# dmMaze/comic-text-detector

Hardware: AMD Instinct MI355X
Metric: pages/sec at 1024x1024 bs=32 (end-to-end detector, device-resident pages) (higher is better)
Workload: dtype f16

## Files before the change

### comic-text-detector_amd/csrc/kernels.h

```cpp
#pragma once
#include <vector>

#include "ctd_common.h"
#include "tuning.h"

void launch_conv_direct(const ConvArgs& a, bool f16, hipStream_t st);
void launch_convt_direct(const ConvArgs& a, bool f16, hipStream_t st);
void launch_input_nchw(const float* in, void* dst, int pitch, int B, int H, int W, bool f16, hipStream_t st);
void launch_input_u8(const uint8_t* in, void* dst, int pitch, int B, int H, int W, bool f16, hipStream_t st);
void launch_maxpool(const void* src, int pitchS, void* dst, int pitchD, int C, int B, int H, int W, int k,
                    bool f16, hipStream_t st);
bool sppf_pool3_supported(int pitch, int slot, int C, int H, int W, int k, const void* cat, int esize = 2);
void launch_sppf_pool3(void* cat, int pitch, int slot, int C, int B, int H, int W, int k, hipStream_t st, int esize = 2);
void launch_avgpool2(const void* src, int pitchS, void* dst, int pitchD, int C, int B, int Ho, int Wo,
                     bool f16, hipStream_t st);
void launch_detect_decode(const void* raw, int pitch, bool raw_f16, float* blks, int rows_total, int row_off,
                          int B, int ny, int nx, int na, int no, float stride, const float* anchors_px,
                          hipStream_t st);
void launch_export_plane(const void* src, int pitch, bool f16, float* out, int nplanes, int plane, uint8_t* u8,
                         int u8_mode, float thresh, int B, int H, int W, hipStream_t st);

void launch_db_step(const float* lines, float k, float* out, uint8_t* bitmap, float thresh, int B, int H, int W,
                    hipStream_t st);

extern int g_igemm_force_bk;
int igemm_pick_bk(int c0, int c1, int K, int N, int log2_down);
void igemm_pack_weights(const float* logical, int nphase, int N, int K, int bn, int bk, bool tiled,
                        std::vector<half_t>& out);
bool igemm_supported(const ConvArgs& a);
int igemm_ntile(int N);
const char* launch_conv_igemm(const ConvArgs& a, bool dst_f32, hipStream_t st);

int f32_mfma_ntile(int N);
bool conv_f32_mfma_supported(const ConvArgs& a);
void launch_conv_f32_mfma(const ConvArgs& a, hipStream_t st);

bool conv_split_supported(const ConvArgs& a);
const char* launch_conv_split(const ConvArgs& a, hipStream_t st);
bool stem_split_supported(const ConvArgs& a);
void launch_stem_split(const ConvArgs& a, const void* input, int in_fmt, hipStream_t st);
bool conv_split_halo_supported(const ConvArgs& a);
void launch_conv_split_halo(const ConvArgs& a, hipStream_t st);
void split_pack_weights(const float* logical, int nphase, int N, int K, int npad, std::vector<half_t>& out,
                        std::vector<float>& oscale);

bool conv_halo_supported(const ConvArgs& a, bool dst_f32);
void launch_conv_halo(const ConvArgs& a, hipStream_t st);

bool conv_halo3_supported(const ConvArgs& a, bool dst_f32);
bool conv_halo3_post_supported(const ConvArgs& a);
bool conv_halo3_segp_supported(const ConvArgs& a);
void launch_conv_halo3(const ConvArgs& a, hipStream_t st);

struct C3Args {
  SrcView s0, s1;
  int B, H, W;
  const half_t *w12, *wm1, *wm2, *wc3;
  const float *b12, *bm1, *bm2, *bc3;
// ... 99 lines not shown
```

### comic-text-detector_amd/csrc/kernels_basic.hip

```cpp
#include "kernels.h"

namespace {

template <typename T>
__device__ __forceinline__ const T* src_pixel(const SrcView& s, int b, int iy, int ix) {
  int sy = s.up ? (iy >> 1) : iy;
  int sx = s.up ? (ix >> 1) : ix;
  return (const T*)s.ptr + ((size_t)((size_t)b * s.H + sy) * s.W + sx) * s.pitch;
}

template <typename T, bool PRECISE>
__global__ __launch_bounds__(256) void conv_direct_kernel(ConvArgs a) {
  const long long total = (long long)a.M * a.N;
  const int Ct = a.s0.c + a.s1.c;
  const float* __restrict__ w = (const float*)a.w;
  for (long long idx = (long long)blockIdx.x * blockDim.x + threadIdx.x; idx < total;
       idx += (long long)gridDim.x * blockDim.x) {
    const int n = (int)(idx % a.N);
    const int m = (int)(idx / a.N);
    const int ox = m % a.Mw;
    const int oy = (m / a.Mw) % a.Mh;
    const int b = m / (a.Mw * a.Mh);
    float acc = 0.f;
    for (int ty = 0; ty < a.KH; ++ty) {
// ... 108 lines not shown
    dst[pix * pitchD + c] = from_f<T>(m);
  }
}

__global__ void maxpool_h8_kernel(const half_t* __restrict__ src, int pitchS, half_t* __restrict__ dst, int pitchD,
                                  int C8, int B, int H, int W, int k) {
  const long long total = (long long)B * H * W * C8;
  const int r = k / 2;
  for (long long i = (long long)blockIdx.x * blockDim.x + threadIdx.x; i < total;
       i += (long long)gridDim.x * blockDim.x) {
    const int c = (int)(i % C8) * 8;
    const long long pix = i / C8;
    const int x = (int)(pix % W), y = (int)((pix / W) % H);
    const long long b = pix / ((long long)W * H);
    half8_t m;
#pragma unroll
    for (int e = 0; e < 8; ++e) m[e] = (half_t)-65504.f;
    for (int dy = -r; dy <= r; ++dy) {
      const int yy = y + dy;
      if (yy < 0 || yy >= H) continue;
      for (int dx = -r; dx <= r; ++dx) {
        const int xx = x + dx;
        if (xx < 0 || xx >= W) continue;
        const half8_t v = *(const half8_t*)(src + ((b * H + yy) * W + xx) * pitchS + c);
#pragma unroll
        for (int e = 0; e < 8; ++e) m[e] = v[e] > m[e] ? v[e] : m[e];
      }
    }
    *(half8_t*)(dst + pix * pitchD + c) = m;
  }
}

constexpr int SPPF_LDS_BYTES = 65536;
template <typename T, typename V, int NV>
__global__ __launch_bounds__(256) void sppf_pool3_kernel(T* __restrict__ cat, int pitch, int slot, int CG, int H, int W, int r) {
  __shared__ __attribute__((aligned(16))) unsigned char sm_raw[SPPF_LDS_BYTES];
  V* A = (V*)sm_raw;
  V* Bf = A + H * W;
  const int HW = H * W;
  const int b = blockIdx.x / CG, cg = blockIdx.x - b * CG;
  T* base = cat + (size_t)b * HW * pitch + cg * NV;
  for (int p = threadIdx.x; p < HW; p += 256) A[p] = *(const V*)(base + (size_t)p * pitch);
  __syncthreads();
  auto vmax = [](V a, V b2) {
    V o;
#pragma unroll
    for (int e = 0; e < NV; ++e) o[e] = b2[e] > a[e] ? b2[e] : a[e];
    return o;
  };
  for (int lvl = 1; lvl <= 3; ++lvl) {
    for (int p = threadIdx.x; p < HW; p += 256) {
      const int y = p / W, x = p - y * W;
      V m = A[p];
      for (int dx = -r; dx <= r; ++dx)
        if (dx && (unsigned)(x + dx) < (unsigned)W) m = vmax(m, A[p + dx]);
      Bf[p] = m;
    }
    __syncthreads();
    for (int p = threadIdx.x; p < HW; p += 256) {
      const int y = p / W;
      V m = Bf[p];
      for (int dy = -r; dy <= r; ++dy)
        if (dy && (unsigned)(y + dy) < (unsigned)H) m = vmax(m, Bf[p + dy * W]);
      A[p] = m;
      *(V*)(base + (size_t)lvl * slot + (size_t)p * pitch) = m;
    }
    __syncthreads();
  }
}

template <typename T>
__global__ void avgpool2_kernel(const T* __restrict__ src, int pitchS, T* __restrict__ dst, int pitchD, int C,
                                int B, int Ho, int Wo) {
  const long long total = (long long)B * Ho * Wo * C;
  const int Wi = Wo * 2, Hi = Ho * 2;
  for (long long i = (long long)blockIdx.x * blockDim.x + threadIdx.x; i < total;
       i += (long long)gridDim.x * blockDim.x) {
    const int c = (int)(i % C);
    const long long pix = i / C;
    const int x = (int)(pix % Wo), y = (int)((pix / Wo) % Ho);
    const long long b = pix / ((long long)Wo * Ho);
    const T* p = src + ((b * Hi + 2 * y) * Wi + 2 * x) * pitchS + c;
    const float s = (to_f(p[0]) + to_f(p[pitchS])) + (to_f(p[(size_t)Wi * pitchS]) + to_f(p[(size_t)(Wi + 1) * pitchS]));
    dst[pix * pitchD + c] = from_f<T>(s * 0.25f);
  }
}

template <typename T>
__global__ void detect_decode_kernel(const T* __restrict__ raw, int pitch, float* __restrict__ blks, int rows_total,
                                     int row_off, int B, int ny, int nx, int na, int no, float stride,
                                     const float* __restrict__ anchors) {
  const long long total = (long long)B * na * ny * nx;
  for (long long i = (long long)blockIdx.x * blockDim.x + threadIdx.x; i < total;
       i += (long long)gridDim.x * blockDim.x) {
    const int x = (int)(i % nx), y = (int)((i / nx) % ny);
    const int an = (int)((i / ((long long)nx * ny)) % na);
    const long long b = i / ((long long)nx * ny * na);
    const T* p = raw + ((b * ny + y) * nx + x) * pitch + an * no;
    float* o = blks + (b * rows_total + row_off + ((long long)an * ny + y) * nx + x) * no;
    for (int j = 0; j < no; ++j) {
      const float s = 1.0f / (1.0f + expf(-to_f(p[j])));
      float v = s;
      if (j == 0) v = (s * 2.f - 0.5f + (float)x) * stride;
      else if (j == 1) v = (s * 2.f - 0.5f + (float)y) * stride;
      else if (j == 2) { const float t = s * 2.f; v = t * t * anchors[an * 2 + 0]; }
      else if (j == 3) { const float t = s * 2.f; v = t * t * anchors[an * 2 + 1]; }
      o[j] = v;
    }
  }
}

template <typename T>
__global__ void export_plane_kernel(const T* __restrict__ src, int pitch, float* __restrict__ out, int nplanes,
                                    int plane, uint8_t* __restrict__ u8, int u8_mode, float thresh, int B, int H,
                                    int W) {
  const long long hw = (long long)H * W;
  const long long total = (long long)B * hw;
  for (long long i = (long long)blockIdx.x * blockDim.x + threadIdx.x; i < total;
       i += (long long)gridDim.x * blockDim.x) {
    const long long b = i / hw, p = i % hw;
    const float v = to_f(src[i * pitch]);
    if (out) out[(b * nplanes + plane) * hw + p] = v;
    if (u8_mode == 1) u8[i] = (uint8_t)(v * 255.0f);
    else if (u8_mode == 2) u8[i] = v > thresh ? 1 : 0;
  }
}

inline int grid_for(long long total, int block = 256) {
  long long g = (total + block - 1) / block;
  if (g > 256LL * 32) g = 256LL * 32;
  if (g < 1) g = 1;
  return (int)g;
}

}

void launch_conv_direct(const ConvArgs& a, bool f16, hipStream_t st) {
  const int g = grid_for((long long)a.M * a.N);
  if (f16) hipLaunchKernelGGL((conv_direct_kernel<half_t, false>), dim3(g), dim3(256), 0, st, a);
  else hipLaunchKernelGGL((conv_direct_kernel<float, true>), dim3(g), dim3(256), 0, st, a);
// ... 6 lines not shown
}

void launch_input_nchw(const float* in, void* dst, int pitch, int B, int H, int W, bool f16, hipStream_t st) {
  const int g = grid_for((long long)B * H * W);
  if (f16) hipLaunchKernelGGL((input_nchw_kernel<half_t>), dim3(g), dim3(256), 0, st, in, (half_t*)dst, pitch, B, H, W);
  else hipLaunchKernelGGL((input_nchw_kernel<float>), dim3(g), dim3(256), 0, st, in, (float*)dst, pitch, B, H, W);
}

void launch_input_u8(const uint8_t* in, void* dst, int pitch, int B, int H, int W, bool f16, hipStream_t st) {
  const long long t = (long long)B * H * W;
  const int g = grid_for(t);
  if (f16) hipLaunchKernelGGL((input_u8_kernel<half_t>), dim3(g), dim3(256), 0, st, in, (half_t*)dst, pitch, t);
  else hipLaunchKernelGGL((input_u8_kernel<float>), dim3(g), dim3(256), 0, st, in, (float*)dst, pitch, t);
}

void launch_maxpool(const void* src, int pitchS, void* dst, int pitchD, int C, int B, int H, int W, int k,
                    bool f16, hipStream_t st) {
  const int g = grid_for((long long)B * H * W * C);
  if (f16 && C % 8 == 0 && pitchS % 8 == 0 && pitchD % 8 == 0 && (((uintptr_t)src | (uintptr_t)dst) & 15) == 0)
    hipLaunchKernelGGL(maxpool_h8_kernel, dim3(grid_for((long long)B * H * W * (C / 8))), dim3(256), 0, st,
                       (const half_t*)src, pitchS, (half_t*)dst, pitchD, C / 8, B, H, W, k);
  else if (f16)
    hipLaunchKernelGGL((maxpool_kernel<half_t>), dim3(g), dim3(256), 0, st, (const half_t*)src, pitchS,
                       (half_t*)dst, pitchD, C, B, H, W, k);
  else
    hipLaunchKernelGGL((maxpool_kernel<float>), dim3(g), dim3(256), 0, st, (const float*)src, pitchS, (float*)dst,
                       pitchD, C, B, H, W, k);
}

bool sppf_pool3_supported(int pitch, int slot, int C, int H, int W, int k, const void* cat, int esize) {
  if (k != 5 && k != 3 && k != 7) return false;
  const int v = 16 / esize;
  if (C % v || pitch % v || slot % v || ((uintptr_t)cat & 15)) return false;
  return (long long)H * W * 2 * 8 <= SPPF_LDS_BYTES;
}
void launch_sppf_pool3(void* cat, int pitch, int slot, int C, int B, int H, int W, int k, hipStream_t st, int esize) {
  typedef float float2_t __attribute__((ext_vector_type(2)));
  const bool wide = (long long)H * W * 2 * 16 <= SPPF_LDS_BYTES;
  if (esize == 4) {
    if (wide)
      hipLaunchKernelGGL((sppf_pool3_kernel<float, float4_t, 4>), dim3(B * (C / 4)), dim3(256), 0, st, (float*)cat, pitch, slot, C / 4, H, W, k / 2);
    else
      hipLaunchKernelGGL((sppf_pool3_kernel<float, float2_t, 2>), dim3(B * (C / 2)), dim3(256), 0, st, (float*)cat, pitch, slot, C / 2, H, W, k / 2);
  } else if (wide) {
    hipLaunchKernelGGL((sppf_pool3_kernel<half_t, half8_t, 8>), dim3(B * (C / 8)), dim3(256), 0, st, (half_t*)cat, pitch, slot, C / 8, H, W, k / 2);
  } else {
    hipLaunchKernelGGL((sppf_pool3_kernel<half_t, half4_t, 4>), dim3(B * (C / 4)), dim3(256), 0, st, (half_t*)cat, pitch, slot, C / 4, H, W, k / 2);
  }
}

void launch_avgpool2(const void* src, int pitchS, void* dst, int pitchD, int C, int B, int Ho, int Wo, bool f16,
                     hipStream_t st) {
  const int g = grid_for((long long)B * Ho * Wo * C);
  if (f16)
    hipLaunchKernelGGL((avgpool2_kernel<half_t>), dim3(g), dim3(256), 0, st, (const half_t*)src, pitchS,
                       (half_t*)dst, pitchD, C, B, Ho, Wo);
  else
    hipLaunchKernelGGL((avgpool2_kernel<float>), dim3(g), dim3(256), 0, st, (const float*)src, pitchS, (float*)dst,
                       pitchD, C, B, Ho, Wo);
}

void launch_detect_decode(const void* raw, int pitch, bool raw_f16, float* blks, int rows_total, int row_off, int B,
                          int ny, int nx, int na, int no, float stride, const float* anchors_px, hipStream_t st) {
  const int g = grid_for((long long)B * na * ny * nx);
  if (raw_f16)
    hipLaunchKernelGGL((detect_decode_kernel<half_t>), dim3(g), dim3(256), 0, st, (const half_t*)raw, pitch, blks,
                       rows_total, row_off, B, ny, nx, na, no, stride, anchors_px);
  else
    hipLaunchKernelGGL((detect_decode_kernel<float>), dim3(g), dim3(256), 0, st, (const float*)raw, pitch, blks,
                       rows_total, row_off, B, ny, nx, na, no, stride, anchors_px);
}

__global__ void db_step_kernel(const float* __restrict__ lines, float k, float* __restrict__ out,
                               uint8_t* __restrict__ bitmap, float thresh, int B, int hw) {
  const long long total = (long long)B * hw;
  for (long long i = (long long)blockIdx.x * blockDim.x + threadIdx.x; i < total; i += (long long)gridDim.x * blockDim.x) {
    const long long b = i / hw, p = i % hw;
    const float x = lines[(b * 2) * hw + p], y = lines[(b * 2 + 1) * hw + p];
    const float v = 1.0f / (1.0f + expf(-k * (x - y)));
    out[i] = v;
    if (bitmap) bitmap[i] = v > thresh ? 1 : 0;
  }
}

void launch_db_step(const float* lines, float k, float* out, uint8_t* bitmap, float thresh, int B, int H, int W,
                    hipStream_t st) {
  hipLaunchKernelGGL(db_step_kernel, dim3(grid_for((long long)B * H * W)), dim3(256), 0, st, lines, k, out, bitmap, thresh,
                     B, H * W);
}

void launch_export_plane(const void* src, int pitch, bool f16, float* out, int nplanes, int plane, uint8_t* u8,
                         int u8_mode, float thresh, int B, int H, int W, hipStream_t st) {
  const int g = grid_for((long long)B * H * W);
  if (!u8) u8_mode = 0;
  if (f16)
    hipLaunchKernelGGL((export_plane_kernel<half_t>), dim3(g), dim3(256), 0, st, (const half_t*)src, pitch, out,
                       nplanes, plane, u8, u8_mode, thresh, B, H, W);
  else
    hipLaunchKernelGGL((export_plane_kernel<float>), dim3(g), dim3(256), 0, st, (const float*)src, pitch, out,
                       nplanes, plane, u8, u8_mode, thresh, B, H, W);
}
```

### comic-text-detector_amd/csrc/kernels_igemm.hip

```cpp
#include <type_traits>
#include <vector>

#include "kernels.h"

namespace {

template <int BN, int BM, int WGN, int WGM, int BK, bool DST_F32, int MINW, int PF>
__global__ __launch_bounds__(256, MINW) void conv_igemm_kernel(ConvArgs a) {
  if (a.prio) __builtin_amdgcn_s_setprio(3);
  constexpr int LP = BK;
  constexpr int SEGS = BK / 8;
  constexpr int RPP = 256 / SEGS;
  constexpr int TN = BN / (32 * WGN);
  constexpr int TM = BM / (32 * WGM);
  constexpr int AROWS = BM / RPP;
  constexpr int WCHUNKS = BN * SEGS;
  constexpr int WROWS = (WCHUNKS + 255) / 256;
  static_assert(WGN * WGM == 4, "4 waves");

  constexpr int LDS_STAGE = 2 * (BM + BN) * LP, LDS_OUT = BM * (BN + 8);
  constexpr int LDS_MAIN = LDS_STAGE > LDS_OUT ? LDS_STAGE : LDS_OUT;
  __shared__ __attribute__((aligned(16))) half_t lds[LDS_MAIN + 2 * BN];
  float* bias_s = (float*)(lds + LDS_MAIN);
  half_t* As = lds;
// ... 322 lines not shown
    for (int it = 0; it < NIT; ++it) {
      const int m = m0 + it * PPI + t / CPP;
      okp[it] = m < a.M && n < a.N;
      opx[it] = okp[it] ? out_pixel(m) : 0;
    }
    if (a.res) {
      half8_t rv[NIT];
#pragma unroll
      for (int it = 0; it < NIT; ++it)
        rv[it] = *(const half8_t*)((const half_t*)a.res + opx[it] * a.pitchR + (okp[it] ? n : 0));
#pragma unroll
      for (int it = 0; it < NIT; ++it) {
        const half8_t o = *(const half8_t*)(Os + (size_t)(it * PPI + t / CPP) * OP + c * 8);
        half8_t sum;
#pragma unroll
        for (int e = 0; e < 8; ++e) sum[e] = (half_t)((float)o[e] + (float)rv[it][e]);
        if (okp[it]) *(half8_t*)((half_t*)a.dst + opx[it] * a.pitchD + n) = sum;
      }
    } else {
#pragma unroll
      for (int it = 0; it < NIT; ++it)
        if (okp[it])
          *(half8_t*)((half_t*)a.dst + opx[it] * a.pitchD + n) = *(const half8_t*)(Os + (size_t)(it * PPI + t / CPP) * OP + c * 8);
    }
  }
}

template <int BN, int BM, int WGN, int WGM, int BK>
void launch_cfg(const ConvArgs& a, bool dst_f32, hipStream_t st) {
  const int ntn = a.Npad / BN;
  const int ntm = (a.M + BM - 1) / BM;
  dim3 grid(ntn * ntm * a.nphase, 1, 1);
  constexpr int HI = BK == 32 ? 4 : 2;
  if (dst_f32) {
    hipLaunchKernelGGL((conv_igemm_kernel<BN, BM, WGN, WGM, BK, true, HI, 1>), grid, dim3(256), 0, st, a);
  } else {
    hipLaunchKernelGGL((conv_igemm_kernel<BN, BM, WGN, WGM, BK, false, HI, 2>), grid, dim3(256), 0, st, a);
  }
}

__global__ void mfma_probe_kernel(const half_t* __restrict__ A, const half_t* __restrict__ B, float* __restrict__ D) {
  const int lane = threadIdx.x;
  const int l31 = lane & 31, kg = (lane >> 5) * 8;
  half8_t fa, fb;
  for (int e = 0; e < 8; ++e) {
    fa[e] = A[l31 * 16 + kg + e];
    fb[e] = B[(kg + e) * 32 + l31];
  }
  float16_t acc;
  for (int r = 0; r < 16; ++r) acc[r] = 0.f;
  acc = __builtin_amdgcn_mfma_f32_32x32x16_f16(fa, fb, acc, 0, 0, 0);
  for (int r = 0; r < 16; ++r) {
    const int row = (r & 3) + 8 * (r >> 2) + 4 * (lane >> 5);
    D[row * 32 + l31] = acc[r];
  }
}

}

int igemm_ntile(int N) {
  if (N % 128 == 0) return 128;
  if (N % 64 == 0) return 64;
  return 32;
}

int g_igemm_force_bk = 0;

int igemm_pick_bk(int c0, int c1, int K, int N, int log2_down) {
  const bool can64 = (c0 % 64 == 0) && (c1 % 64 == 0);
  if (g_igemm_force_bk == 32 || !can64) return 32;
  if (g_igemm_force_bk == 64) return 64;
// ... 7 lines not shown
  const int Npad = (N + bn - 1) / bn * bn;
  const int nk = K / bk;
  out.assign((size_t)nphase * Npad * K, (half_t)0.f);
  for (int ph = 0; ph < nphase; ++ph)
    for (int n = 0; n < N; ++n) {
      const float* src = logical + ((size_t)ph * N + n) * K;
      for (int k = 0; k < K; ++k) {
        size_t dst;
        if (tiled)
          dst = (size_t)ph * Npad * K + ((((size_t)(n / bn) * nk + k / bk) * bn + n % bn) * bk + k % bk);
        else
          dst = ((size_t)ph * Npad + n) * K + k;
        out[dst] = (half_t)src[k];
      }
    }
}

bool igemm_supported(const ConvArgs& a) {
  constexpr int BK = 32;
  if (a.s0.c % BK || a.s1.c % BK) return false;
  if (a.s0.pitch % 8 || (a.s1.c && a.s1.pitch % 8)) return false;
  if (a.pitchD % 4 || (a.res && a.pitchR % 4)) return false;
  if (a.K % BK) return false;
  return true;
}

static void magic_div(int d, unsigned& mul, unsigned& sh) {
  int L = 0;
  while ((1ll << L) < d) ++L;
  sh = 31 + L;
  mul = (unsigned)(((1ull << sh) / (unsigned)d) + 1);
}

const char* launch_conv_igemm(const ConvArgs& a_in, bool dst_f32, hipStream_t st) {
  ConvArgs a = a_in;
  magic_div(a.Mw, a.mw_mul, a.mw_sh);
  magic_div(a.Mh, a.mh_mul, a.mh_sh);
  a.bk = pick_bk(a);
  if (conv_halo3_supported(a, dst_f32)) { launch_conv_halo3(a, st); return "conv_halo3_kernel"; }
  if (conv_halo_supported(a, dst_f32)) { launch_conv_halo(a, st); return "conv_halo_kernel"; }
  const int bn = igemm_ntile(a.N);
  if (pick_bk(a) == 64) {
    if (bn == 128) launch_cfg<128, 128, 2, 2, 64>(a, dst_f32, st);
    else if (bn == 64) launch_cfg<64, 128, 2, 2, 64>(a, dst_f32, st);
    else launch_cfg<32, 128, 1, 4, 64>(a, dst_f32, st);
  } else {
    if (bn == 128) launch_cfg<128, 128, 2, 2, 32>(a, dst_f32, st);
    else if (bn == 64) launch_cfg<64, 128, 2, 2, 32>(a, dst_f32, st);
    else launch_cfg<32, 128, 1, 4, 32>(a, dst_f32, st);
  }
  return "conv_igemm_kernel";
}

void launch_mfma_probe(const half_t* a, const half_t* b, float* out, hipStream_t st) {
  hipLaunchKernelGGL(mfma_probe_kernel, dim3(1), dim3(64), 0, st, a, b, out);
}
```

### comic-text-detector_amd/csrc/selftest.hip

```cpp
#include <cmath>
#include <cstdio>
#include <cstdlib>
#include <cstring>
#include <string>
#include <vector>

#include "kernels.h"

#define CK(x)                                                                              \
  do {                                                                                     \
    hipError_t e_ = (x);                                                                   \
    if (e_ != hipSuccess) {                                                                \
      std::printf("HIP error %s at %s:%d\n", hipGetErrorString(e_), __FILE__, __LINE__);   \
      std::exit(2);                                                                        \
    }                                                                                      \
  } while (0)

static unsigned g_seed = 12345;
static float frand() {
  static const bool zero = std::getenv("ST_ZERO") != nullptr;
  g_seed = g_seed * 1664525u + 1013904223u;
  return zero ? 0.f : ((g_seed >> 8) & 0xFFFF) / 65536.0f - 0.5f;
}

template <typename T>
static T* dev_alloc(size_t n) {
  T* p;
  CK(hipMalloc((void**)&p, n * sizeof(T) + 64));
  return p;
}

static int g_fail = 0;

static void probe() {
  std::vector<half_t> A(32 * 16), B(16 * 32);
  for (auto& v : A) v = (half_t)frand();
// ... 1038 lines not shown
    size_t bad = 0;
    for (size_t i = 0; i < nout; ++i) {
      const double e = std::fabs((double)o[i] - (double)r[i]);
      maxd = std::fmax(maxd, e / (1.0 + std::fabs((double)r[i])));
      if (!(e <= 2e-5 * (1.0 + std::fabs((double)r[i])))) ++bad;
    }
    if (bad) ++g_fail;
    std::printf(" %s: %s max|d| %.2e (%zu > 2e-5)", var == 0 ? "u8->f32" : var == 1 ? "u8->planes" : "nchw->f32", bad ? "FAIL" : "ok", maxd, bad);
  }
  if (timing) {
    hipEvent_t e0, e1;
    CK(hipEventCreate(&e0)); CK(hipEventCreate(&e1));
    auto tm = [&](auto&& fn) {
      for (int i = 0; i < 3; ++i) fn();
      CK(hipEventRecord(e0, 0));
      for (int i = 0; i < 20; ++i) fn();
      CK(hipEventRecord(e1, 0));
      CK(hipEventSynchronize(e1));
      float ms;
      CK(hipEventElapsedTime(&ms, e0, e1));
      return ms / 20;
    };
    an.d_sp = 1;
    const float t_new = tm([&]() { launch_stem_split(an, dImg, CTD_IN_NHWC_U8, 0); });
    const float t_old = tm([&]() { launch_input_u8(dImg, dIn4, 4, B, H, W, false, 0); launch_conv_split(a, 0); });
    std::printf(" | INPUT + generic %.3f ms, from the page %.3f ms (%.0f GB/s of its bytes)", t_old, t_new,
                ((double)npx * 3 + (double)nout * 4) / (t_new * 1e-3) / 1e9);
  }
  std::printf("\n");
  (void)hipFree(dImg); (void)hipFree(dPl); (void)hipFree(dIn4); (void)hipFree(dWs); (void)hipFree(dBias); (void)hipFree(dOsc);
  (void)hipFree(dRef); (void)hipFree(dOut);
}

int main(int argc, char** argv) {
  const int B = argc > 1 ? std::atoi(argv[1]) : 4;
  const bool quick = argc > 2;
  char name[256];
  int cus = 0;
  int64_t hbm = 0;
  const int arch = ctd_device_info(0, name, &cus, &hbm);
  std::printf("device: %s gfx%d CUs=%d HBM=%.1f GB\n", name, arch, cus, hbm / 1e9);
  if (const char* tu = std::getenv("CTD_TUNING")) {
    std::string s(tu);
    for (size_t p = 0; p < s.size();) {
      const size_t e = s.find(',', p), q = s.find('=', p);
      const size_t end = e == std::string::npos ? s.size() : e;
      if (q != std::string::npos && q < end) {
        const std::string k = s.substr(p, q - p);
        const long long v = std::atoll(s.substr(q + 1, end - q - 1).c_str());
        std::printf("tuning %s = %lld: %s\n", k.c_str(), v, ctd_tuning_set(k.c_str(), v) == CTD_OK ? "ok" : "UNKNOWN KEY");
      }
      p = end + 1;
    }
  }
  probe();
  const Case cases[] = {
      {"1x1 64->64 @256 (N64)", 0, 64, 0, 0, 64, 1, 1, 256, 0},
      {"1x1 32->32 @256 (N32)", 0, 32, 0, 0, 32, 1, 1, 256, 0},
      {"1x1 128->21 @128 detect (N21)", 0, 128, 0, 0, 21, 1, 1, 128, 0},
      {"1x1 256->256 @128", 0, 256, 0, 0, 256, 1, 1, 128, 0},
      {"1x1 512->512 @64", 0, 512, 0, 0, 512, 1, 1, 64, 0},
      {"1x1 cat(256up,256)->256 @64", 0, 256, 256, 1, 256, 1, 1, 64, 0},
      {"1x1 cat(512,256)->512 @32", 0, 512, 256, 0, 512, 1, 1, 32, 0},
      {"1x1 cat(128,256)->256 @128", 0, 128, 256, 0, 256, 1, 1, 128, 0},
      {"3x3 32->32 @256 +res", 0, 32, 0, 0, 32, 3, 1, 256, 1},
      {"3x3 64->64 @128 +res", 0, 64, 0, 0, 64, 3, 1, 128, 1},
      {"3x3 128->128 @128 +res", 0, 128, 0, 0, 128, 3, 1, 128, 1},
      {"3x3 256->256 @64 +res", 0, 256, 0, 0, 256, 3, 1, 64, 1},
      {"3x3 64->32 @256 (db tail)", 0, 64, 0, 0, 32, 3, 1, 256, 0},
      {"3x3s2 32->64 @512", 0, 32, 0, 0, 64, 3, 2, 512, 0},
      {"3x3s2 64->128 @256", 0, 64, 0, 0, 128, 3, 2, 256, 0},
      {"3x3s2 256->512 @64", 0, 256, 0, 0, 512, 3, 2, 64, 0},
      {"convT4 512->256 @64", 1, 512, 0, 0, 256, 4, 2, 64, 0},
      {"convT4 256->128 @128", 1, 256, 0, 0, 128, 4, 2, 128, 0},
      {"convT4 128->64 @256", 1, 128, 0, 0, 64, 4, 2, 256, 0},
      {"convT4 512->256 @16", 1, 512, 0, 0, 256, 4, 2, 16, 0},
  };
  const int ncase = sizeof(cases) / sizeof(cases[0]);
  if (std::getenv("ST_CORUN")) {
    run_stem2_case("1024x1024 pages", B, 1024, 1024, CTD_IN_NHWC_U8, CTD_ACT_SILU);
    std::printf("selftest: %s (%d failures)\n", g_fail ? "FAILED" : "PASSED", g_fail);
    return g_fail ? 1 : 0;
  }
  if (std::getenv("ST_SPLIT")) {
    probe_denorm();
    const Case ragged[] = {{"3x3 32->64 @20 ragged (s2)", 0, 32, 0, 0, 64, 3, 2, 20, 0},
                           {"1x1 cat(32up,64)->21 @12", 0, 32, 64, 1, 21, 1, 1, 12, 0},
                           {"convT4 64->32 @9", 1, 64, 0, 0, 32, 4, 2, 9, 0},
                           {"3x3 64->16 @24 (db branch)", 0, 64, 0, 0, 16, 3, 1, 24, 0},
                           {"stem 6x6s2 4->32 @44 ragged", 0, 4, 0, 0, 32, 6, 2, 44, 0},
                           {"3x3 64->64 @21 +res", 0, 64, 0, 0, 64, 3, 1, 21, 1},
                           {"3x3 cat(32,32)->128 @18 (halo)", 0, 32, 32, 0, 128, 3, 1, 18, 0},
                           {"convT4 64->64 @19 (halo)", 1, 64, 0, 0, 64, 4, 2, 19, 0},
                           {"convT4 96->128 @33 (halo)", 1, 96, 0, 0, 128, 4, 2, 33, 0}};
    for (const Case& c : ragged) run_split_case(c, 3, false);
    run_stem_split_case(3, 88, false);
    run_stem_split_case(B, 1024, true);
    run_split_case(Case{"stem 6x6s2 4->32 @1024", 0, 4, 0, 0, 32, 6, 2, 1024, 0}, B, true);
    const char* sel = std::getenv("ST_CASES");
    for (int i = 0; i < ncase; ++i) {
      if (sel) {
        bool on = false;
        for (const char* p = sel; *p;) {
          if (std::atoi(p) == i) on = true;
          while (*p && *p != ',') ++p;
          if (*p == ',') ++p;
        }
        if (!on) continue;
      }
      run_split_case(cases[i], B, true);
    }
    std::printf("selftest: %s (%d failures)\n", g_fail ? "FAILED" : "PASSED", g_fail);
    return g_fail ? 1 : 0;
  }
  if (!std::getenv("ST_NO_C3")) {
    const C3Case c3s[] = {{"model.2 (64 -> 64 @256)", 64, 0, 256, CTD_ACT_SILU},
// ... 49 lines not shown
```

Baseline: 3373.

## Retune small-map kernels: BM64 igemm for small grids, regroup SPPF, vectorize pools and decode

Adds a BM=64 igemm tile path, used when the BM=128 grid would have fewer than two blocks per CU, so small late-stage feature maps fill more of the device. The SPPF pool kernel now runs 512 threads, packs several channel groups per block, keeps intermediates in registers with dynamic LDS, and always uses 16-byte vectors. avgpool2 gets a vectorized path, and detect_decode stages raw rows in LDS so its output writes are contiguous. Selftests check each path bit-exact against reference kernels. The risk is the extra kernel instantiations and a CU-count heuristic that may not suit every layer.

After: 3397, median of 6. No clear change (+0.7%).

```diff
diff --git a/comic-text-detector_amd/csrc/kernels.h b/comic-text-detector_amd/csrc/kernels.h
--- a/comic-text-detector_amd/csrc/kernels.h
+++ b/comic-text-detector_amd/csrc/kernels.h
@@ -24,6 +24,7 @@
                     hipStream_t st);
 
 extern int g_igemm_force_bk;
+extern int g_igemm_force_bm;
 int igemm_pick_bk(int c0, int c1, int K, int N, int log2_down);
 void igemm_pack_weights(const float* logical, int nphase, int N, int K, int bn, int bk, bool tiled,
                         std::vector<half_t>& out);
diff --git a/comic-text-detector_amd/csrc/kernels_basic.hip b/comic-text-detector_amd/csrc/kernels_basic.hip
--- a/comic-text-detector_amd/csrc/kernels_basic.hip
+++ b/comic-text-detector_amd/csrc/kernels_basic.hip
@@ -164,80 +164,132 @@
 }
 
 constexpr int SPPF_LDS_BYTES = 65536;
+constexpr int SPPF_THREADS = 512, SPPF_EPT = 8;
 template <typename T, typename V, int NV>
-__global__ __launch_bounds__(256) void sppf_pool3_kernel(T* __restrict__ cat, int pitch, int slot, int CG, int H, int W, int r) {
-  __shared__ __attribute__((aligned(16))) unsigned char sm_raw[SPPF_LDS_BYTES];
-  V* A = (V*)sm_raw;
-  V* Bf = A + H * W;
-  const int HW = H * W;
-  const int b = blockIdx.x / CG, cg = blockIdx.x - b * CG;
-  T* base = cat + (size_t)b * HW * pitch + cg * NV;
-  for (int p = threadIdx.x; p < HW; p += 256) A[p] = *(const V*)(base + (size_t)p * pitch);
-  __syncthreads();
+__global__ __launch_bounds__(SPPF_THREADS) void sppf_pool3_kernel(T* __restrict__ cat, int pitch, int slot, int CG, int G, int H,
+                                                                  int W, int r) {
+  extern __shared__ __attribute__((aligned(16))) unsigned char sppf_raw[];
+  V* A = (V*)sppf_raw;
+  const int E = H * W * G, WG = W * G;
+  const int nblk = (CG + G - 1) / G;
+  const int b = blockIdx.x / nblk, cg0 = (blockIdx.x - b * nblk) * G;
+  const int gn = CG - cg0 < G ? CG - cg0 : G;
+  T* base = cat + (size_t)b * H * W * pitch + cg0 * NV;
   auto vmax = [](V a, V b2) {
     V o;
 #pragma unroll
     for (int e = 0; e < NV; ++e) o[e] = b2[e] > a[e] ? b2[e] : a[e];
     return o;
   };
+  int goff[SPPF_EPT], px[SPPF_EPT], py[SPPF_EPT];
+  bool on[SPPF_EPT];
+  V m[SPPF_EPT];
+#pragma unroll
+  for (int k = 0; k < SPPF_EPT; ++k) {
+    const int i = threadIdx.x + k * SPPF_THREADS;
+    const int p = i / G, g = i - p * G;
+    on[k] = i < E && g < gn;
+    py[k] = p / W;
+    px[k] = p - py[k] * W;
+    goff[k] = p * pitch + g * NV;
+    if (on[k]) A[i] = *(const V*)(base + goff[k]);
+  }
+  __syncthreads();
   for (int lvl = 1; lvl <= 3; ++lvl) {
-    for (int p = threadIdx.x; p < HW; p += 256) {
-      const int y = p / W, x = p - y * W;
-      V m = A[p];
+#pragma unroll
+    for (int k = 0; k < SPPF_EPT; ++k) {
+      const int i = threadIdx.x + k * SPPF_THREADS;
+      if (!on[k]) continue;
+      m[k] = A[i];
       for (int dx = -r; dx <= r; ++dx)
-        if (dx && (unsigned)(x + dx) < (unsigned)W) m = vmax(m, A[p + dx]);
-      Bf[p] = m;
+        if (dx && (unsigned)(px[k] + dx) < (unsigned)W) m[k] = vmax(m[k], A[i + dx * G]);
     }
     __syncthreads();
-    for (int p = threadIdx.x; p < HW; p += 256) {
-      const int y = p / W;
-      V m = Bf[p];
+#pragma unroll
+    for (int k = 0; k < SPPF_EPT; ++k)
+      if (on[k]) A[threadIdx.x + k * SPPF_THREADS] = m[k];
+    __syncthreads();
+#pragma unroll
+    for (int k = 0; k < SPPF_EPT; ++k) {
+      const int i = threadIdx.x + k * SPPF_THREADS;
+      if (!on[k]) continue;
+      m[k] = A[i];
       for (int dy = -r; dy <= r; ++dy)
-        if (dy && (unsigned)(y + dy) < (unsigned)H) m = vmax(m, Bf[p + dy * W]);
-      A[p] = m;
-      *(V*)(base + (size_t)lvl * slot + (size_t)p * pitch) = m;
-    }
+        if (dy && (unsigned)(py[k] + dy) < (unsigned)H) m[k] = vmax(m[k], A[i + dy * WG]);
+      *(V*)(base + (size_t)lvl * slot + goff[k]) = m[k];
+    }
+    if (lvl == 3) break;
     __syncthreads();
-  }
-}
-
-template <typename T>
+#pragma unroll
+    for (int k = 0; k < SPPF_EPT; ++k)
+      if (on[k]) A[threadIdx.x + k * SPPF_THREADS] = m[k];
+    __syncthreads();
+  }
+}
+
+template <typename T, int NV>
 __global__ void avgpool2_kernel(const T* __restrict__ src, int pitchS, T* __restrict__ dst, int pitchD, int C,
                                 int B, int Ho, int Wo) {
-  const long long total = (long long)B * Ho * Wo * C;
+  typedef T V __attribute__((ext_vector_type(NV)));
+  const int CV = C / NV;
+  const long long total = (long long)B * Ho * Wo * CV;
   const int Wi = Wo * 2, Hi = Ho * 2;
   for (long long i = (long long)blockIdx.x * blockDim.x + threadIdx.x; i < total;
        i += (long long)gridDim.x * blockDim.x) {
-    const int c = (int)(i % C);
-    const long long pix = i / C;
+    const int c = (int)(i % CV) * NV;
+    const long long pix = i / CV;
     const int x = (int)(pix % Wo), y = (int)((pix / Wo) % Ho);
     const long long b = pix / ((long long)Wo * Ho);
     const T* p = src + ((b * Hi + 2 * y) * Wi + 2 * x) * pitchS + c;
-    const float s = (to_f(p[0]) + to_f(p[pitchS])) + (to_f(p[(size_t)Wi * pitchS]) + to_f(p[(size_t)(Wi + 1) * pitchS]));
-    dst[pix * pitchD + c] = from_f<T>(s * 0.25f);
-  }
-}
-
-template <typename T>
-__global__ void detect_decode_kernel(const T* __restrict__ raw, int pitch, float* __restrict__ blks, int rows_total,
-                                     int row_off, int B, int ny, int nx, int na, int no, float stride,
-                                     const float* __restrict__ anchors) {
-  const long long total = (long long)B * na * ny * nx;
-  for (long long i = (long long)blockIdx.x * blockDim.x + threadIdx.x; i < total;
-       i += (long long)gridDim.x * blockDim.x) {
-    const int x = (int)(i % nx), y = (int)((i / nx) % ny);
-    const int an = (int)((i / ((long long)nx * ny)) % na);
-    const long long b = i / ((long long)nx * ny * na);
-    const T* p = raw + ((b * ny + y) * nx + x) * pitch + an * no;
-    float* o = blks + (b * rows_total + row_off + ((long long)an * ny + y) * nx + x) * no;
-    for (int j = 0; j < no; ++j) {
-      const float s = 1.0f / (1.0f + expf(-to_f(p[j])));
-      float v = s;
-      if (j == 0) v = (s * 2.f - 0.5f + (float)x) * stride;
-      else if (j == 1) v = (s * 2.f - 0.5f + (float)y) * stride;
-      else if (j == 2) { const float t = s * 2.f; v = t * t * anchors[an * 2 + 0]; }
-      else if (j == 3) { const float t = s * 2.f; v = t * t * anchors[an * 2 + 1]; }
-      o[j] = v;
+    if constexpr (NV == 1) {
+      const float s = (to_f(p[0]) + to_f(p[pitchS])) + (to_f(p[(size_t)Wi * pitchS]) + to_f(p[(size_t)(Wi + 1) * pitchS]));
+      dst[pix * pitchD + c] = from_f<T>(s * 0.25f);
+    } else {
+      const V p0 = *(const V*)p, p1 = *(const V*)(p + pitchS);
+      const V p2 = *(const V*)(p + (size_t)Wi * pitchS), p3 = *(const V*)(p + (size_t)(Wi + 1) * pitchS);
+      V o;
+#pragma unroll
+      for (int e = 0; e < NV; ++e) {
+        const float s = (to_f(p0[e]) + to_f(p1[e])) + (to_f(p2[e]) + to_f(p3[e]));
+        o[e] = from_f<T>(s * 0.25f);
+      }
+      *(V*)(dst + pix * pitchD + c) = o;
+    }
+  }
+}
+
+__device__ __forceinline__ float detect_decode_elem(float raw, int j, int x, int y, int an, float stride,
+                                                    const float* __restrict__ anchors) {
+  const float s = 1.0f / (1.0f + expf(-raw));
+  float v = s;
+  if (j == 0) v = (s * 2.f - 0.5f + (float)x) * stride;
+  else if (j == 1) v = (s * 2.f - 0.5f + (float)y) * stride;
+  else if (j == 2) { const float t = s * 2.f; v = t * t * anchors[an * 2 + 0]; }
+  else if (j == 3) { const float t = s * 2.f; v = t * t * anchors[an * 2 + 1]; }
+  return v;
+}
+
+template <typename T>
+__global__ __launch_bounds__(256) void detect_decode_kernel(const T* __restrict__ raw, int pitch, float* __restrict__ blks,
+                                                            int rows_total, int row_off, int chunks, int P, int ny, int nx,
+                                                            int na, int no, float stride, const float* __restrict__ anchors) {
+  extern __shared__ __attribute__((aligned(16))) float dd_raw[];
+  const int hw = ny * nx, nano = na * no;
+  const int b = blockIdx.x / chunks, q0 = (blockIdx.x - b * chunks) * P;
+  const int np = hw - q0 < P ? hw - q0 : P;
+  const T* src = raw + ((size_t)b * hw + q0) * pitch;
+  for (int i = threadIdx.x; i < np * nano; i += 256) {
+    const int p = i / nano, c = i - p * nano;
+    dd_raw[i] = to_f(src[(size_t)p * pitch + c]);
+  }
+  __syncthreads();
+  const int run = np * no;
+  for (int an = 0; an < na; ++an) {
+    float* o = blks + ((size_t)b * rows_total + row_off + (size_t)an * hw + q0) * no;
+    for (int i = threadIdx.x; i < run; i += 256) {
+      const int p = i / no, j = i - p * no;
+      const int q = q0 + p, y = q / nx, x = q - y * nx;
+      o[i] = detect_decode_elem(dd_raw[p * nano + an * no + j], j, x, y, an, stride, anchors);
     }
   }
 }
@@ -310,43 +362,54 @@
   if (k != 5 && k != 3 && k != 7) return false;
   const int v = 16 / esize;
   if (C % v || pitch % v || slot % v || ((uintptr_t)cat & 15)) return false;
-  return (long long)H * W * 2 * 8 <= SPPF_LDS_BYTES;
+  return (long long)H * W * 16 <= SPPF_LDS_BYTES;
 }
 void launch_sppf_pool3(void* cat, int pitch, int slot, int C, int B, int H, int W, int k, hipStream_t st, int esize) {
-  typedef float float2_t __attribute__((ext_vector_type(2)));
-  const bool wide = (long long)H * W * 2 * 16 <= SPPF_LDS_BYTES;
-  if (esize == 4) {
-    if (wide)
-      hipLaunchKernelGGL((sppf_pool3_kernel<float, float4_t, 4>), dim3(B * (C / 4)), dim3(256), 0, st, (float*)cat, pitch, slot, C / 4, H, W, k / 2);
-    else
-      hipLaunchKernelGGL((sppf_pool3_kernel<float, float2_t, 2>), dim3(B * (C / 2)), dim3(256), 0, st, (float*)cat, pitch, slot, C / 2, H, W, k / 2);
-  } else if (wide) {
-    hipLaunchKernelGGL((sppf_pool3_kernel<half_t, half8_t, 8>), dim3(B * (C / 8)), dim3(256), 0, st, (half_t*)cat, pitch, slot, C / 8, H, W, k / 2);
-  } else {
-    hipLaunchKernelGGL((sppf_pool3_kernel<half_t, half4_t, 4>), dim3(B * (C / 4)), dim3(256), 0, st, (half_t*)cat, pitch, slot, C / 4, H, W, k / 2);
-  }
+  static_assert(SPPF_THREADS * SPPF_EPT * 16 <= SPPF_LDS_BYTES, "a block's entries: one plane in LDS, one pass in registers");
+  const int CG = C / (16 / esize);
+  int G = 1;
+  while (G < 4 && G * 2 <= CG && (long long)H * W * G * 2 <= SPPF_THREADS * SPPF_EPT) G *= 2;
+  const int nblk = (CG + G - 1) / G;
+  const size_t lds = (size_t)H * W * G * 16;
+  if (esize == 4)
+    hipLaunchKernelGGL((sppf_pool3_kernel<float, float4_t, 4>), dim3(B * nblk), dim3(SPPF_THREADS), lds, st, (float*)cat, pitch, slot, CG, G, H, W, k / 2);
+  else
+    hipLaunchKernelGGL((sppf_pool3_kernel<half_t, half8_t, 8>), dim3(B * nblk), dim3(SPPF_THREADS), lds, st, (half_t*)cat, pitch, slot, CG, G, H, W, k / 2);
 }
 
 void launch_avgpool2(const void* src, int pitchS, void* dst, int pitchD, int C, int B, int Ho, int Wo, bool f16,
                      hipStream_t st) {
-  const int g = grid_for((long long)B * Ho * Wo * C);
-  if (f16)
-    hipLaunchKernelGGL((avgpool2_kernel<half_t>), dim3(g), dim3(256), 0, st, (const half_t*)src, pitchS,
+  const int v = f16 ? 8 : 4;
+  const bool wide = C % v == 0 && pitchS % v == 0 && pitchD % v == 0 && (((uintptr_t)src | (uintptr_t)dst) & 15) == 0;
+  const int g = grid_for((long long)B * Ho * Wo * (wide ? C / v : C));
+  if (f16 && wide)
+    hipLaunchKernelGGL((avgpool2_kernel<half_t, 8>), dim3(g), dim3(256), 0, st, (const half_t*)src, pitchS,
                        (half_t*)dst, pitchD, C, B, Ho, Wo);
+  else if (f16)
+    hipLaunchKernelGGL((avgpool2_kernel<half_t, 1>), dim3(g), dim3(256), 0, st, (const half_t*)src, pitchS,
+                       (half_t*)dst, pitchD, C, B, Ho, Wo);
+  else if (wide)
+    hipLaunchKernelGGL((avgpool2_kernel<float, 4>), dim3(g), dim3(256), 0, st, (const float*)src, pitchS, (float*)dst,
+                       pitchD, C, B, Ho, Wo);
   else
-    hipLaunchKernelGGL((avgpool2_kernel<float>), dim3(g), dim3(256), 0, st, (const float*)src, pitchS, (float*)dst,
+    hipLaunchKernelGGL((avgpool2_kernel<float, 1>), dim3(g), dim3(256), 0, st, (const float*)src, pitchS, (float*)dst,
                        pitchD, C, B, Ho, Wo);
 }
 
 void launch_detect_decode(const void* raw, int pitch, bool raw_f16, float* blks, int rows_total, int row_off, int B,
                           int ny, int nx, int na, int no, float stride, const float* anchors_px, hipStream_t st) {
-  const int g = grid_for((long long)B * na * ny * nx);
+  if (B <= 0 || ny <= 0 || nx <= 0 || na <= 0 || no <= 0) return;
+  const int nano = na * no;
+  int P = 12288 / nano;
+  P = P > 64 ? 64 : P < 1 ? 1 : P;
+  const int chunks = (ny * nx + P - 1) / P;
+  const size_t lds = (size_t)P * nano * sizeof(float);
   if (raw_f16)
-    hipLaunchKernelGGL((detect_decode_kernel<half_t>), dim3(g), dim3(256), 0, st, (const half_t*)raw, pitch, blks,
-                       rows_total, row_off, B, ny, nx, na, no, stride, anchors_px);
+    hipLaunchKernelGGL((detect_decode_kernel<half_t>), dim3(B * chunks), dim3(256), lds, st, (const half_t*)raw, pitch, blks,
+                       rows_total, row_off, chunks, P, ny, nx, na, no, stride, anchors_px);
   else
-    hipLaunchKernelGGL((detect_decode_kernel<float>), dim3(g), dim3(256), 0, st, (const float*)raw, pitch, blks,
-                       rows_total, row_off, B, ny, nx, na, no, stride, anchors_px);
+    hipLaunchKernelGGL((detect_decode_kernel<float>), dim3(B * chunks), dim3(256), lds, st, (const float*)raw, pitch, blks,
+                       rows_total, row_off, chunks, P, ny, nx, na, no, stride, anchors_px);
 }
 
 __global__ void db_step_kernel(const float* __restrict__ lines, float k, float* __restrict__ out,
diff --git a/comic-text-detector_amd/csrc/kernels_igemm.hip b/comic-text-detector_amd/csrc/kernels_igemm.hip
--- a/comic-text-detector_amd/csrc/kernels_igemm.hip
+++ b/comic-text-detector_amd/csrc/kernels_igemm.hip
@@ -378,11 +378,13 @@
   const int ntm = (a.M + BM - 1) / BM;
   dim3 grid(ntn * ntm * a.nphase, 1, 1);
   constexpr int HI = BK == 32 ? 4 : 2;
-  if (dst_f32) {
-    hipLaunchKernelGGL((conv_igemm_kernel<BN, BM, WGN, WGM, BK, true, HI, 1>), grid, dim3(256), 0, st, a);
-  } else {
-    hipLaunchKernelGGL((conv_igemm_kernel<BN, BM, WGN, WGM, BK, false, HI, 2>), grid, dim3(256), 0, st, a);
-  }
+  if constexpr (BM == 128) {
+    if (dst_f32) {
+      hipLaunchKernelGGL((conv_igemm_kernel<BN, BM, WGN, WGM, BK, true, HI, 1>), grid, dim3(256), 0, st, a);
+      return;
+    }
+  }
+  hipLaunchKernelGGL((conv_igemm_kernel<BN, BM, WGN, WGM, BK, false, HI, 2>), grid, dim3(256), 0, st, a);
 }
 
 __global__ void mfma_probe_kernel(const half_t* __restrict__ A, const half_t* __restrict__ B, float* __restrict__ D) {
@@ -456,6 +458,23 @@
   mul = (unsigned)(((1ull << sh) / (unsigned)d) + 1);
 }
 
+int g_igemm_force_bm = 0;
+
+#ifndef IGEMM_SMALL_GRID_CUS
+#define IGEMM_SMALL_GRID_CUS 2
+#endif
+static bool igemm_small_grid(const ConvArgs& a, int bn) {
+  if (g_igemm_force_bm) return g_igemm_force_bm == 64;
+  static const int cus = [] {
+    int dev = 0, n = 0;
+    if (hipGetDevice(&dev) != hipSuccess || hipDeviceGetAttribute(&n, hipDeviceAttributeMultiprocessorCount, dev) != hipSuccess || n <= 0)
+      n = 256;
+    return n;
+  }();
+  const long long grid128 = (long long)(a.Npad / bn) * ((a.M + 127) / 128) * a.nphase;
+  return grid128 < (long long)IGEMM_SMALL_GRID_CUS * cus;
+}
+
 const char* launch_conv_igemm(const ConvArgs& a_in, bool dst_f32, hipStream_t st) {
   ConvArgs a = a_in;
   magic_div(a.Mw, a.mw_mul, a.mw_sh);
@@ -464,7 +483,18 @@
   if (conv_halo3_supported(a, dst_f32)) { launch_conv_halo3(a, st); return "conv_halo3_kernel"; }
   if (conv_halo_supported(a, dst_f32)) { launch_conv_halo(a, st); return "conv_halo_kernel"; }
   const int bn = igemm_ntile(a.N);
-  if (pick_bk(a) == 64) {
+  const bool bk64 = pick_bk(a) == 64;
+  if (bn != 32 && !dst_f32 && igemm_small_grid(a, bn)) {
+    if (bk64) {
+      if (bn == 128) launch_cfg<128, 64, 2, 2, 64>(a, false, st);
+      else launch_cfg<64, 64, 2, 2, 64>(a, false, st);
+    } else {
+      if (bn == 128) launch_cfg<128, 64, 2, 2, 32>(a, false, st);
+      else launch_cfg<64, 64, 2, 2, 32>(a, false, st);
+    }
+    return "conv_igemm_kernel";
+  }
+  if (bk64) {
     if (bn == 128) launch_cfg<128, 128, 2, 2, 64>(a, dst_f32, st);
     else if (bn == 64) launch_cfg<64, 128, 2, 2, 64>(a, dst_f32, st);
     else launch_cfg<32, 128, 1, 4, 64>(a, dst_f32, st);
diff --git a/comic-text-detector_amd/csrc/selftest.hip b/comic-text-detector_amd/csrc/selftest.hip
--- a/comic-text-detector_amd/csrc/selftest.hip
+++ b/comic-text-detector_amd/csrc/selftest.hip
@@ -2,6 +2,7 @@
 #include <cstdio>
 #include <cstdlib>
 #include <cstring>
+#include <functional>
 #include <string>
 #include <vector>
 
@@ -1106,6 +1107,252 @@
   (void)hipFree(dRef); (void)hipFree(dOut);
 }
 
+template <typename T>
+static std::vector<T> from_dev(const T* d, size_t n) {
+  std::vector<T> h(n);
+  CK(hipMemcpy(h.data(), d, n * sizeof(T), hipMemcpyDeviceToHost));
+  return h;
+}
+template <typename T>
+static T* to_dev(const std::vector<T>& h) {
+  T* d = dev_alloc<T>(h.size());
+  CK(hipMemcpy(d, h.data(), h.size() * sizeof(T), hipMemcpyHostToDevice));
+  return d;
+}
+static double time_ms(int it, const std::function<void()>& f) {
+  hipEvent_t e0, e1;
+  CK(hipEventCreate(&e0)); CK(hipEventCreate(&e1));
+  f();
+  CK(hipEventRecord(e0, 0));
+  for (int i = 0; i < it; ++i) f();
+  CK(hipEventRecord(e1, 0));
+  CK(hipEventSynchronize(e1));
+  float t;
+  CK(hipEventElapsedTime(&t, e0, e1));
+  CK(hipEventDestroy(e0)); CK(hipEventDestroy(e1));
+  return t / it;
+}
+
+struct TileCase { const char* name; int c0, c1, up0, N, k, s, H, W, res, bk; };
+static void run_tile_case(const TileCase& cs, int B) {
+  const int cin = cs.c0 + cs.c1, k = cs.k, s = cs.s, pad = k / 2;
+  const int Ho = (cs.H + 2 * pad - k) / s + 1, Wo = (cs.W + 2 * pad - k) / s + 1;
+  const int H0 = cs.up0 ? cs.H / 2 : cs.H, W0 = cs.up0 ? cs.W / 2 : cs.W;
+  std::vector<half_t> h0((size_t)B * H0 * W0 * cs.c0), h1(cs.c1 ? (size_t)B * cs.H * cs.W * cs.c1 : 1);
+  for (auto& v : h0) v = (half_t)frand();
+  for (auto& v : h1) v = (half_t)frand();
+  half_t *d0 = to_dev(h0), *d1 = to_dev(h1);
+  const size_t nout = (size_t)B * Ho * Wo * cs.N;
+  half_t *dOut = dev_alloc<half_t>(nout), *dRef = dev_alloc<half_t>(nout), *dRes = nullptr;
+  if (cs.res) {
+    std::vector<half_t> hr(nout);
+    for (auto& v : hr) v = (half_t)frand();
+    dRes = to_dev(hr);
+  }
+  const int bn = igemm_ntile(cs.N), K = k * k * cin;
+  const float wscale = 1.0f / std::sqrt((float)K);
+  std::vector<float> lg((size_t)cs.N * K), wdr((size_t)K * cs.N), bias(cs.N);
+  for (int n = 0; n < cs.N; ++n)
+    for (int kk = 0; kk < K; ++kk) {
+      const float w = (float)(half_t)(frand() * 2.f * wscale);
+      lg[(size_t)n * K + kk] = w;
+      wdr[(size_t)kk * cs.N + n] = w;
+    }
+  for (auto& v : bias) v = frand();
+  float *dBias = to_dev(bias), *dWdr = to_dev(wdr);
+  static void* zeros = nullptr;
+  if (!zeros) { CK(hipMalloc(&zeros, CTD_ZEROS_BYTES)); CK(hipMemset(zeros, 0, CTD_ZEROS_BYTES)); }
+  ConvArgs a{};
+  a.s0 = SrcView{d0, cs.c0, cs.c0, cs.up0, H0, W0};
+  if (cs.c1) a.s1 = SrcView{d1, cs.c1, cs.c1, 0, cs.H, cs.W};
+  a.B = B; a.Hin = cs.H; a.Win = cs.W; a.bias = dBias; a.pitchD = cs.N; a.oH = Ho; a.oW = Wo;
+  a.res = dRes; a.pitchR = cs.N; a.act = CTD_ACT_SILU; a.N = cs.N; a.nphase = 1; a.osy = a.osx = 1; a.zeros = zeros;
+  a.Mh = Ho; a.Mw = Wo; a.KH = a.KW = k; a.stride = s; a.dy0 = a.dx0 = -pad; a.K = K; a.M = B * Ho * Wo;
+  ConvArgs ig = a, dr = a;
+  dr.w = dWdr; dr.Npad = cs.N; dr.dst = dRef;
+  launch_conv_direct(dr, true, 0);
+  const int bk = cs.bk ? cs.bk : igemm_pick_bk(cs.c0, cs.c1, K, cs.N, 0);
+  std::vector<half_t> wig;
+  igemm_pack_weights(lg.data(), 1, cs.N, K, bn, bk, true, wig);
+  half_t* dWig = to_dev(wig);
+  ig.w = dWig; ig.Npad = (cs.N + bn - 1) / bn * bn; ig.dst = dOut; ig.bk = bk; ig.w_tiled = 1;
+  const int halo = g_conv_halo;
+  const long long halo3 = g_halo3;
+  g_conv_halo = 0; g_halo3 = 0;
+  std::vector<half_t> o[2];
+  double ms[2];
+  bool sup = igemm_supported(ig);
+  for (int v = 0; v < 2 && sup; ++v) {
+    g_igemm_force_bm = v ? 128 : 64;
+    CK(hipMemset(dOut, 0xff, nout * 2));
+    launch_conv_igemm(ig, false, 0);
+    CK(hipDeviceSynchronize());
+    o[v] = from_dev(dOut, nout);
+    ms[v] = time_ms(10, [&] { launch_conv_igemm(ig, false, 0); });
+  }
+  g_igemm_force_bm = 0; g_conv_halo = halo; g_halo3 = halo3;
+  const std::vector<half_t> r = from_dev(dRef, nout);
+  size_t diff = 0, bad = 0;
+  for (size_t i = 0; i < nout && sup; ++i) {
+    if (std::memcmp(&o[0][i], &o[1][i], 2) != 0) ++diff;
+    const double e = std::fabs((double)o[0][i] - (double)r[i]);
+    if (!(e <= 4e-3 * (1.0 + std::fabs((double)r[i])))) ++bad;
+  }
+  const bool ok = sup && !diff && !bad;
+  if (!ok) ++g_fail;
+  std::printf("[igemm-tile] %-34s B=%d M=%d N=%d K=%d bk=%d | 64-pixel tile %.4f ms, 128-pixel tile %.4f ms | %zu of %zu differ, %zu beyond "
+              "tolerance of the direct kernel | %s\n", cs.name, B, a.M, cs.N, K, bk, sup ? ms[0] : 0., sup ? ms[1] : 0., diff, nout, bad,
+              ok ? "ok(bit-exact)" : "FAIL");
+  (void)hipFree(d0); (void)hipFree(d1); (void)hipFree(dOut); (void)hipFree(dRef); if (dRes) (void)hipFree(dRes);
+  (void)hipFree(dBias); (void)hipFree(dWdr); (void)hipFree(dWig);
+}
+
+template <typename T>
+static void run_sppf2_case(int B, int H, int W, int C) {
+  const bool f16 = sizeof(T) == 2;
+  std::vector<T> h((size_t)B * H * W * 4 * C);
+  for (auto& v : h) v = (T)frand();
+  T *dA = to_dev(h), *dB = to_dev(h);
+  const bool sup = sppf_pool3_supported(4 * C, C, C, H, W, 5, dB, sizeof(T));
+  for (int j = 0; j < 3; ++j) launch_maxpool(dA + j * C, 4 * C, dA + (j + 1) * C, 4 * C, C, B, H, W, 5, f16, 0);
+  if (sup) launch_sppf_pool3(dB, 4 * C, C, C, B, H, W, 5, 0, sizeof(T));
+  CK(hipDeviceSynchronize());
+  const std::vector<T> a = from_dev(dA, h.size()), b = from_dev(dB, h.size());
+  const bool ok = sup && std::memcmp(a.data(), b.data(), h.size() * sizeof(T)) == 0;
+  if (!ok) ++g_fail;
+  const double ms = sup ? time_ms(10, [&] { launch_sppf_pool3(dB, 4 * C, C, C, B, H, W, 5, 0, sizeof(T)); }) : 0.;
+  std::printf("[sppf2] %s B=%d %dx%d C=%d | fused %.4f ms | %s\n", f16 ? "fp16" : "f32", B, H, W, C, ms,
+              !sup ? "unsupported FAIL" : ok ? "ok(bit-exact)" : "FAIL");
+  (void)hipFree(dA); (void)hipFree(dB);
+}
+
+template <typename T>
+__global__ void ref_detect_decode_kernel(const T* __restrict__ raw, int pitch, float* __restrict__ blks, int rows_total,
+                                         int row_off, int B, int ny, int nx, int na, int no, float stride,
+                                         const float* __restrict__ anchors) {
+  const long long total = (long long)B * na * ny * nx;
+  for (long long i = (long long)blockIdx.x * blockDim.x + threadIdx.x; i < total;
+       i += (long long)gridDim.x * blockDim.x) {
+    const int x = (int)(i % nx), y = (int)((i / nx) % ny);
+    const int an = (int)((i / ((long long)nx * ny)) % na);
+    const long long b = i / ((long long)nx * ny * na);
+    const T* p = raw + ((b * ny + y) * nx + x) * pitch + an * no;
+    float* o = blks + (b * rows_total + row_off + ((long long)an * ny + y) * nx + x) * no;
+    for (int j = 0; j < no; ++j) {
+      const float s = 1.0f / (1.0f + expf(-to_f(p[j])));
+      float v = s;
+      if (j == 0) v = (s * 2.f - 0.5f + (float)x) * stride;
+      else if (j == 1) v = (s * 2.f - 0.5f + (float)y) * stride;
+      else if (j == 2) { const float t = s * 2.f; v = t * t * anchors[an * 2 + 0]; }
+      else if (j == 3) { const float t = s * 2.f; v = t * t * anchors[an * 2 + 1]; }
+      o[j] = v;
+    }
+  }
+}
+template <typename T>
+__global__ void ref_avgpool2_kernel(const T* __restrict__ src, int pitchS, T* __restrict__ dst, int pitchD, int C,
+                                    int B, int Ho, int Wo) {
+  const long long total = (long long)B * Ho * Wo * C;
+  const int Wi = Wo * 2, Hi = Ho * 2;
+  for (long long i = (long long)blockIdx.x * blockDim.x + threadIdx.x; i < total;
+       i += (long long)gridDim.x * blockDim.x) {
+    const int c = (int)(i % C);
+    const long long pix = i / C;
+    const int x = (int)(pix % Wo), y = (int)((pix / Wo) % Ho);
+    const long long b = pix / ((long long)Wo * Ho);
+    const T* p = src + ((b * Hi + 2 * y) * Wi + 2 * x) * pitchS + c;
+    const float s = (to_f(p[0]) + to_f(p[pitchS])) + (to_f(p[(size_t)Wi * pitchS]) + to_f(p[(size_t)(Wi + 1) * pitchS]));
+    dst[pix * pitchD + c] = from_f<T>(s * 0.25f);
+  }
+}
+
+template <typename T>
+static void run_decode_case(int B, int ny, int nx) {
+  const int na = 3, no = 7, pitch = 24, row_off = 5, rows_total = na * ny * nx + 9;
+  std::vector<T> h((size_t)B * ny * nx * pitch);
+  for (auto& v : h) v = (T)(frand() * 12.f);
+  const std::vector<float> anchors = {10.f, 13.f, 16.5f, 30.f, 33.f, 23.25f};
+  T* dRaw = to_dev(h);
+  float* dAn = to_dev(anchors);
+  const size_t nblk = (size_t)B * rows_total * no;
+  float *dA = dev_alloc<float>(nblk), *dB = dev_alloc<float>(nblk);
+  CK(hipMemset(dA, 0xff, nblk * 4)); CK(hipMemset(dB, 0xff, nblk * 4));
+  const long long rows = (long long)B * na * ny * nx;
+  hipLaunchKernelGGL((ref_detect_decode_kernel<T>), dim3((unsigned)((rows + 255) / 256)), dim3(256), 0, 0, dRaw, pitch, dA, rows_total,
+                     row_off, B, ny, nx, na, no, 8.f, dAn);
+  launch_detect_decode(dRaw, pitch, sizeof(T) == 2, dB, rows_total, row_off, B, ny, nx, na, no, 8.f, dAn, 0);
+  CK(hipDeviceSynchronize());
+  const std::vector<float> a = from_dev(dA, nblk), b = from_dev(dB, nblk);
+  size_t diff = 0;
+  for (size_t i = 0; i < nblk; ++i) diff += std::memcmp(&a[i], &b[i], 4) != 0;
+  if (diff) ++g_fail;
+  std::printf("[decode] %s B=%d %dx%d na=%d no=%d (%lld elements) | %zu of %zu differ | %s\n", sizeof(T) == 2 ? "fp16" : "f32", B, ny, nx,
+              na, no, rows * no, diff, nblk, diff ? "FAIL" : "ok(bit-exact)");
+  (void)hipFree(dRaw); (void)hipFree(dAn); (void)hipFree(dA); (void)hipFree(dB);
+}
+
+template <typename T>
+static void run_avgpool_case(int B, int Ho, int Wo, int C) {
+  const int pitchS = C + 8, pitchD = C + 16;
+  std::vector<T> h((size_t)B * 4 * Ho * Wo * pitchS);
+  for (auto& v : h) v = (T)frand();
+  T* dS = to_dev(h);
+  const size_t nd = (size_t)B * Ho * Wo * pitchD;
+  T *dA = dev_alloc<T>(nd), *dB = dev_alloc<T>(nd);
+  CK(hipMemset(dA, 0xff, nd * sizeof(T))); CK(hipMemset(dB, 0xff, nd * sizeof(T)));
+  const long long tot = (long long)B * Ho * Wo * C;
+  hipLaunchKernelGGL((ref_avgpool2_kernel<T>), dim3((unsigned)((tot + 255) / 256)), dim3(256), 0, 0, dS, pitchS, dA, pitchD, C, B, Ho, Wo);
+  launch_avgpool2(dS, pitchS, dB, pitchD, C, B, Ho, Wo, sizeof(T) == 2, 0);
+  CK(hipDeviceSynchronize());
+  const std::vector<T> a = from_dev(dA, nd), b = from_dev(dB, nd);
+  const bool ok = std::memcmp(a.data(), b.data(), nd * sizeof(T)) == 0;
+  if (!ok) ++g_fail;
+  std::printf("[avgpool] %s B=%d out %dx%d C=%d | %s\n", sizeof(T) == 2 ? "fp16" : "f32", B, Ho, Wo, C, ok ? "ok(bit-exact)" : "FAIL");
+  (void)hipFree(dS); (void)hipFree(dA); (void)hipFree(dB);
+}
+
+static void run_smallmap(int B) {
+  const TileCase tiles[] = {
+      {"1x1 256->256 @16", 256, 0, 0, 256, 1, 1, 16, 16, 0, 0},
+      {"1x1 cat(256up,128)->256 @16", 256, 128, 1, 256, 1, 1, 16, 16, 0, 0},
+      {"3x3 128->128 @16 +res", 128, 0, 0, 128, 3, 1, 16, 16, 1, 0},
+      {"3x3s2 256->512 @16 -> 8x8", 256, 0, 0, 512, 3, 2, 16, 16, 0, 0},
+      {"1x1 128->64 @16 (bn 64)", 128, 0, 0, 64, 1, 1, 16, 16, 0, 0},
+      {"1x1 512->256 @16 (bk 64)", 512, 0, 0, 256, 1, 1, 16, 16, 0, 64},
+      {"3x3 64->64 @16 +res (bn 64, bk 64)", 64, 0, 0, 64, 3, 1, 16, 16, 1, 64},
+  };
+  for (const TileCase& c : tiles) run_tile_case(c, B > 3 ? 3 : B);
+  run_tile_case(TileCase{"3x3 64->128 on 5x7, M=105", 64, 0, 0, 128, 3, 1, 5, 7, 0, 0}, 3);
+  run_tile_case(TileCase{"1x1 64->128 on 5x7 +res, M=105", 64, 0, 0, 128, 1, 1, 5, 7, 1, 0}, 3);
+  run_tile_case(TileCase{"3x3 32->64 on 1x43, M=129", 32, 0, 0, 64, 3, 1, 1, 43, 0, 0}, 3);
+  run_tile_case(TileCase{"1x1 64->256 on 5x13, M=65", 64, 0, 0, 256, 1, 1, 5, 13, 0, 0}, 1);
+  run_sppf2_case<half_t>(B, 2, 2, 64);
+  run_sppf2_case<half_t>(B, 5, 3, 64);
+  run_sppf2_case<half_t>(B, 32, 32, 256);
+  run_sppf2_case<half_t>(B, 48, 48, 64);
+  run_sppf2_case<half_t>(B, 5, 3, 8);
+  run_sppf2_case<half_t>(B, 16, 16, 40);
+  run_sppf2_case<half_t>(B, 32, 32, 24);
+  run_sppf2_case<float>(B, 2, 2, 64);
+  run_sppf2_case<float>(B, 32, 32, 64);
+  run_sppf2_case<float>(B, 48, 48, 16);
+  run_sppf2_case<float>(B, 5, 3, 4);
+  run_sppf2_case<float>(B, 16, 16, 20);
+  for (int b : {1, 3}) {
+    run_decode_case<float>(b, 3, 5);
+    run_decode_case<float>(b, 16, 16);
+    run_decode_case<half_t>(b, 3, 5);
+    run_decode_case<half_t>(b, 16, 16);
+  }
+  run_decode_case<float>(2, 9, 13);
+  for (int C : {8, 24, 20}) {
+    run_avgpool_case<half_t>(B, 4, 5, C);
+    run_avgpool_case<float>(B, 4, 5, C);
+  }
+  run_avgpool_case<half_t>(B, 16, 16, 64);
+  run_avgpool_case<float>(B, 3, 7, 6);
+}
+
 int main(int argc, char** argv) {
   const int B = argc > 1 ? std::atoi(argv[1]) : 4;
   const bool quick = argc > 2;
@@ -1156,6 +1403,11 @@
     std::printf("selftest: %s (%d failures)\n", g_fail ? "FAILED" : "PASSED", g_fail);
     return g_fail ? 1 : 0;
   }
+  if (std::getenv("ST_SMALLMAP")) {
+    run_smallmap(B);
+    std::printf("selftest: %s (%d failures)\n", g_fail ? "FAILED" : "PASSED", g_fail);
+    return g_fail ? 1 : 0;
+  }
   if (std::getenv("ST_SPLIT")) {
     probe_denorm();
     const Case ragged[] = {{"3x3 32->64 @20 ragged (s2)", 0, 32, 0, 0, 64, 3, 2, 20, 0},
```
